# feihuzhang/GANet

Measured on AMD Instinct MI355X. Metric: cost-volumes/sec (SGA+LGA fwd+bwd) at 240x624x192, higher is better.
Workload: dtype f32; 1 GPU; configs[1]: SGA fwd+bwd [1,32,65,80,208] (4x guidance [1,32,5,80,208]) + LGA2 r=2 fwd+bwd [1,193,240,624] (filters [1,75,240,624]), one sample per GPU; parallelism=independent cost volumes per GPU, no data-path collective, launch=hipGraph replay

## Files before the change

### ganet_amd/_native.py

```python
import ctypes
import os
import threading

_HERE = os.path.dirname(os.path.abspath(__file__))
LIB_NAME = "libganet_hip.so"
ABI_VERSION = 11

_P = ctypes.c_void_p
_I = ctypes.c_int

_PROTOS = {
    "ganet_abi_version": [],
    "ganet_is_simulator": [],
    "ganet_set_option": [ctypes.c_char_p, _I],
    "ganet_get_option": [ctypes.c_char_p],
    "ganet_sga_scan_forward": [_P, _P, _P, _I, _I, _I, _I, _I, _I, _P],
    "ganet_sga_forward": [_P] * 9 + [_I] * 5 + [_P],
    "ganet_sga_forward_infer": [_P] * 9 + [_I] * 5 + [_P],
    "ganet_sga_forward_infer_scratch": [_P] * 6 + [_I] * 5,
    "ganet_sga_backward_scan": [_P] * 5 + [_I] * 6 + [_P],
    "ganet_sga_merge": [_P] * 4 + [_I] * 5 + [_P],
    "ganet_sga_scan_forward_ws": [_P] * 3 + [_I] * 6 + [_P],
    "ganet_sga_backward_scan_ws": [_P] * 5 + [_I] * 6 + [_P],
    "ganet_sga_workspace_layout": [_I] * 5,
    "ganet_sga_backward_point": [_P] * 12 + [_I] * 5 + [_P],
    "ganet_sga_backward_dir": [_P] * 9 + [_I] * 7 + [_P],
    "ganet_sga_backward": [_P] * 15 + [_I] * 5 + [_P],
    "ganet_sga_forward_compat": [_P] * 8 + [_I] * 5 + [_P],
    "ganet_sga_backward_compat": [_P] * 15 + [_I] * 5 + [_P],
    "ganet_lga_forward": [_P] * 3 + [_I] * 5 + [_P],
    "ganet_lga_backward": [_P] * 5 + [_I] * 6 + [_P],
    "ganet_lga_forward_regress": [_P] * 5 + [_I] * 5 + [_P],
    "ganet_lga_apply_paired": [_P] * 3 + [_I] * 8 + [_P],
    "ganet_lga_apply_paired_edges": [_P] * 4 + [_I] * 8 + [_P],
    "ganet_lga_filter_grad_paired": [_P] * 3 + [_I] * 8 + [_P],
    "ganet_cost_volume_forward": [_P] * 3 + [_I] * 5 + [_P],
    "ganet_cost_volume_backward": [_P] * 3 + [_I] * 5 + [_P],
    "ganet_disparity_regression_forward": [_P] * 2 + [_I] * 4 + [_P],
    "ganet_disparity_regression_backward": [_P] * 2 + [_I] * 4 + [_P],
    "ganet_l1_normalize_forward": [_P] * 5 + [_I] * 6 + [_P],
    "ganet_l1_normalize_backward": [_P] * 6 + [_I] * 6 + [_P],
    "ganet_norm_disparity_regression_forward": [_P] * 3 + [_I] * 4 + [_P],
    "ganet_norm_disparity_regression_backward": [_P] * 5 + [_I] * 4 + [_P],
    "ganet_softmin_forward": [_P] * 2 + [_I] * 4 + [_P],
    "ganet_softmin_backward": [_P] * 3 + [_I] * 4 + [_P],
    "ganet_softmin_regression_forward": [_P] * 4 + [_I] * 4 + [_P],
    "ganet_softmin_regression_backward": [_P] * 6 + [_I] * 4 + [_P],
    "ganet_trilinear_upsample_forward": [_P] * 2 + [_I] * 7 + [_P],
    "ganet_trilinear_upsample_backward": [_P] * 2 + [_I] * 7 + [_P],
    "ganet_residual_relu_forward": [_P] * 5 + [_I] * 5 + [_P],
    "ganet_residual_relu_backward": [_P] * 5 + [_I] * 5 + [_P],
    "ganet_selftest_dpp": [_P, _P, _P],
    "ganet_selftest_dpp_wave": [_P, _P, _P],
}
EXPORTS = sorted(list(_PROTOS) + ["ganet_last_error"])


class GanetError(RuntimeError):

    def __init__(self, message, code=None):
        super().__init__(message)
        self.code = code


E_INVALID, E_UNSUPPORTED, E_RUNTIME = -1, -2, -3


class CApi:
# ... 68 lines not shown
```

### ganet_amd/csrc/ganet_capi.hip

```cpp
#include "ga_common.h"
#include "lga_kernels.h"
#include "misc_kernels.h"
#include "sga_kernels.h"
#include "sga_row_kernels.h"
#include "sga_col_kernels.h"

#include <stdarg.h>
#include <stdio.h>
#include <stdlib.h>
#include <string.h>

#include <atomic>
#include <mutex>

#include "../../include/ganet_hip.h"

#include "ga_launch.h"

namespace {

using namespace ga;

thread_local char g_err[512] = "";

int fail(int code, const char *fmt, ...)
{
  va_list ap;
  va_start(ap, fmt);
  vsnprintf(g_err, sizeof(g_err), fmt, ap);
  va_end(ap);
  return code;
}

int check_launch(const char *what)
{
  const hipError_t e = hipGetLastError();
  if (e != hipSuccess) return fail(GANET_E_RUNTIME, "%s: %s", what, hipGetErrorString(e));
  return GANET_OK;
}

#define GA_TRY(expr)                         \
  do {                                       \
    const int rc_ = (expr);                  \
    if (rc_ != GANET_OK) return rc_;         \
  } while (0)

#define GA_HIP(expr)                                                                   \
  do {                                                                                 \
    const hipError_t e_ = (expr);                                                      \
    if (e_ != hipSuccess) return fail(GANET_E_RUNTIME, #expr ": %s", hipGetErrorString(e_)); \
  } while (0)

#ifndef GA_SGA_TILED_DEFAULT
#define GA_SGA_TILED_DEFAULT 1
#endif
struct Options {
  std::atomic<int> sga_tiled{GA_SGA_TILED_DEFAULT};
  std::atomic<int> lga_wave{2};
  std::atomic<int> lga_mix{1};
  std::atomic<int> lga_segs{0};
  std::atomic<int> wide_col{1};
  std::atomic<int> wide_scan{1};
  std::atomic<int> rowwave{1};
  std::atomic<int> colblock{1};
};
Options g_opt;
std::once_flag g_opt_once;

bool store_option(const char *name, int value)
{
  auto tri = [](int v) { return v < 0 ? 0 : (v > 2 ? 2 : v); };
  if (!strcmp(name, "GANET_LGA_WAVE")) g_opt.lga_wave = tri(value);
  else if (!strcmp(name, "GANET_SGA_TILED")) g_opt.sga_tiled = value ? 1 : 0;
  else if (!strcmp(name, "GANET_LGA_MIX")) g_opt.lga_mix = value < 0 ? 0 : value;
  else if (!strcmp(name, "GANET_LGA_SEGS")) g_opt.lga_segs = value > 0 ? value : 0;
  else if (!strcmp(name, "GANET_SGA_WIDE_SCAN")) g_opt.wide_scan = tri(value);
  else if (!strcmp(name, "GANET_SGA_WIDE_COL")) g_opt.wide_col = tri(value);
  else if (!strcmp(name, "GANET_SGA_ROWWAVE")) g_opt.rowwave = value ? 1 : 0;
  else if (!strcmp(name, "GANET_SGA_COLBLOCK")) g_opt.colblock = value ? 1 : 0;
  else return false;
  return true;
}

void load_env_options()
{
  for (const char *name : {"GANET_LGA_WAVE", "GANET_SGA_TILED", "GANET_LGA_SEGS", "GANET_LGA_MIX", "GANET_SGA_WIDE_SCAN",
                           "GANET_SGA_WIDE_COL", "GANET_SGA_ROWWAVE", "GANET_SGA_COLBLOCK"}) {
    const char *v = getenv(name);
    if (v && *v) store_option(name, atoi(v));
  }
}
const Options &opts()
{
  std::call_once(g_opt_once, load_env_options);
  return g_opt;
}

#define GA_SGA_PAIRS(X) \
  X(16, 1) X(16, 2) X(16, 3) X(16, 5) X(16, 9) X(16, 13) X(16, 17) \
  X(64, 3) X(64, 5) X(64, 9) X(64, 17)

constexpr int fwd_sb(int dpl) { return dpl <= 3 ? 8 : dpl <= 5 ? 4 : dpl <= 9 ? 2 : 1; }
constexpr int fwd_nv(int dpl) { return dpl <= 5 ? 2 : 1; }
constexpr int bwd_sb(int dpl) { return dpl <= 3 ? 8 : dpl <= 5 ? 4 : dpl <= 9 ? 2 : 1; }
constexpr int bwd_nv(int dpl) { return dpl <= 5 ? 2 : 1; }

bool pick_pair(int D, int want_gd, int *gd, int *dpl)
{
  int best_gd = 0, best_dpl = 0;
#define X(G, P)                                                                    \
  if ((G) == want_gd && (G) * (P) >= D && (best_gd == 0 || (P) < best_dpl)) {      \
    best_gd = (G);                                                                 \
    best_dpl = (P);                                                                \
  }
  GA_SGA_PAIRS(X)
#undef X
  if (best_gd == 0 && want_gd == 16) return pick_pair(D, 64, gd, dpl);
  if (best_gd == 0) return false;
  *gd = best_gd;
  *dpl = best_dpl;
// ... 378 lines not shown
    nseg = tiles * 2 > slots ? 1 : (int)((slots + tiles - 1) / tiles);
    if (nseg > D / 16) nseg = D / 16 > 1 ? D / 16 : 1;
  }
  if (nseg > D) nseg = D;
  if (nseg > 1) {
    mx.n_whole = 0;
    mx.sub_len = ((D + nseg - 1) / nseg + 1) & ~1;
    mx.nsub = (D + mx.sub_len - 1) / mx.sub_len;
    *items = tiles * mx.nsub;
    return mx;
  }
  const int mixo = opts().lga_mix;
  const i64 S = mixo > 1 ? (i64)mixo : (i64)units;
  if (mixo && opts().lga_segs <= 0 && tiles / S < LGA_WAVES_PER_SIMD && tiles % S != 0) {
    const i64 r = tiles % S;
    int nsub = (int)(S / r);
    if (nsub > D / 16) nsub = D / 16;
    if (nsub >= 2) {
      mx.n_whole = (int)(tiles - r);
      mx.sub_len = ((D + nsub - 1) / nsub + 1) & ~1;
      mx.nsub = (D + mx.sub_len - 1) / mx.sub_len;
      *items = mx.n_whole + r * mx.nsub;
    }
  }
  return mx;
}

#ifndef GA_LGA_PLANAR
#ifndef GA_FGP_DEFAULT
#define GA_FGP_DEFAULT 1
#endif
#ifndef GA_FGP_WPS
#define GA_FGP_WPS 5
#endif
#define GA_LGA_PLANAR 1
#endif
template <int R>
int launch_lga_fwd(const float *x, const float *f, float *y, int B, int D, int H, int W,
                   bool transposed, hipStream_t st)
{
  LgaGeom geo;
  geo.D = D; geo.H = H; geo.W = W; geo.HW = (i64)H * W;
  if constexpr (R <= 2) {
    const int family = opts().lga_wave;
    if (family && (i64)H * W < (1ll << 28)) {
      i64 items;
      bool planar = false;
      if constexpr (R == 2) planar = GA_LGA_PLANAR && W % 4 == 0 && aligned16(x);
      if constexpr (R == 2) {
        if (planar && family == 2) {
          const LgaSegMix wx = lga_items(W, H, B, D, false, &items, true);
          if (items < (1ll << 31)) {
            if (transposed) GA_LAUNCH((lga_apply_pp_wx<2, true>), dim3((unsigned)items), dim3(256), st, x, f, y, geo, wx);
            else GA_LAUNCH((lga_apply_pp_wx<2, false>), dim3((unsigned)items), dim3(256), st, x, f, y, geo, wx);
            return check_launch("lga apply (plane pairs, workgroup ring)");
          }
        }
      }
      const LgaSegMix mx = lga_items(W, H, B, D, false, &items);
      if (items < (1ll << 31)) {
        if constexpr (R == 2) {
          if (planar && transposed) GA_LAUNCH((lga_apply_pp_x<2, true>), dim3((unsigned)items), dim3(64), st, x, f, y, geo, mx);
          else if (planar) GA_LAUNCH((lga_apply_pp_x<2, false>), dim3((unsigned)items), dim3(64), st, x, f, y, geo, mx);
        }
        if (planar) {}
        else if (transposed) GA_LAUNCH((lga_apply_pp<R, true>), dim3((unsigned)items), dim3(64), st, x, f, y, geo, mx);
// ... 41 lines not shown
#define L(K, T) GA_LAUNCH((K<2, T>), dim3((unsigned)items), dim3(64), st, x, f, y, geo, sg, none, none, edge)
  if (x_paired) {
    if (transposed) L(lga_apply_pp_pi, true); else L(lga_apply_pp_pi, false);
  } else if (GA_LGA_PLANAR && W % 4 == 0) {
    if (transposed) L(lga_apply_pp_xo, true); else L(lga_apply_pp_xo, false);
  } else {
    if (transposed) L(lga_apply_pp_po, true); else L(lga_apply_pp_po, false);
  }
#undef L
  return check_launch("lga apply (plane pairs, interleaved volume)");
}

int launch_lga_gf_paired(const float *x, const float *gy, float *gf, int B, int D, int H, int W, int acc, bool x_paired,
                         hipStream_t st)
{
  if ((i64)H * W >= (1ll << 28) || W % 2 != 0 || !aligned16(x) || !aligned16(gy))
    return fail(GANET_E_UNSUPPORTED, "ganet_lga_filter_grad_paired: needs W even, planes below 2^28 pixels and 16-byte aligned volumes");
  LgaGeom geo;
  geo.D = D; geo.H = H; geo.W = W; geo.HW = (i64)H * W;
  LgaSeg sg;
  sg.tiles_x = (W + LGA_TW - 1) / LGA_TW;
  sg.tiles_y = (H + LGAW_TH - 1) / LGAW_TH;
  sg.nseg = 1; sg.seg_len = D;
  const i64 items = (i64)sg.tiles_x * sg.tiles_y * B;
  if (items >= (1ll << 31)) return fail(GANET_E_UNSUPPORTED, "ganet_lga_filter_grad_paired: too many tiles");
  const bool fg_pair = GA_FGP_DEFAULT && opts().lga_wave >= 2;
  if (x_paired && fg_pair) GA_LAUNCH((lga_filter_grad_pair_xp<GA_FGP_WPS>), dim3((unsigned)items), dim3(128), st, x, gy, gf, geo, sg, acc);
  else if (x_paired) GA_LAUNCH((lga_filter_grad_pp_xp<2, 3, 0>), dim3((unsigned)items), dim3(64), st, x, gy, gf, geo, sg, acc);
  else if (GA_LGA_PLANAR && W % 4 == 0) GA_LAUNCH((lga_filter_grad_pp_gypx<2, 3, 0>), dim3((unsigned)items), dim3(64), st, x, gy, gf, geo, sg, acc);
  else GA_LAUNCH((lga_filter_grad_pp_gyp<2, 3, 0>), dim3((unsigned)items), dim3(64), st, x, gy, gf, geo, sg, acc);
  return check_launch("lga filter grad (plane pairs, interleaved volume)");
}

template <int R>
int launch_lga_fwd_regress(const float *x, const float *f, float *y, float *snorm, float *sdy, int B, int D, int H, int W,
                           hipStream_t st)
{
  if constexpr (R <= 2) {
    if ((i64)H * W < (1ll << 28)) {
      LgaGeom geo;
      geo.D = D; geo.H = H; geo.W = W; geo.HW = (i64)H * W;
      i64 items;
      const LgaSegMix sg = lga_items(W, H, B, D, true, &items);
      if (items < (1ll << 31)) {
        bool planar = false;
        if constexpr (R == 2) {
          planar = GA_LGA_PLANAR && W % 4 == 0 && aligned16(x);
          if (planar) GA_LAUNCH((lga_apply_pp_x<2, false, true>), dim3((unsigned)items), dim3(64), st, x, f, y, geo, sg, snorm, sdy);
        }
        if (!planar) GA_LAUNCH((lga_apply_pp<R, false, true>), dim3((unsigned)items), dim3(64), st, x, f, y, geo, sg, snorm, sdy);
        return check_launch("lga apply + regression epilogue (plane pairs)");
      }
    }
  }
  return fail(GANET_E_UNSUPPORTED, "ganet_lga_forward_regress: no fused kernel for this shape / radius: run ganet_lga_forward "
                                   "and ganet_norm_disparity_regression_forward instead");
}

template <int R>
int launch_lga_gf(const float *x, const float *gy, float *gf, int B, int D, int H, int W, int acc,
                  hipStream_t st)
{
  LgaGeom geo;
  geo.D = D; geo.H = H; geo.W = W; geo.HW = (i64)H * W;
  if constexpr (R <= 2) {
    if (opts().lga_wave && (i64)H * W < (1ll << 28)) {
// ... 48 lines not shown
{
  const int lane = threadIdx.x;
  out[0 * 64 + lane] = dpp_i<DPP_WAVE_SHL1>(-1, lane);
  out[1 * 64 + lane] = dpp_i<DPP_WAVE_SHR1>(-1, lane);
  out[2 * 64 + lane] = (int)seg_allmax<64>((float)((lane * 37) % 64));
  out[3 * 64 + lane] = (int)seg_allsum<64>((float)lane);
}

}

GA_EXPORT int ganet_abi_version(void) { return GANET_ABI_VERSION; }
GA_EXPORT const char *ganet_last_error(void) { return g_err; }
GA_EXPORT int ganet_is_simulator(void)
{
#if defined(GA_HIPSIM)
  return 1;
#else
  return 0;
#endif
}

GA_EXPORT int ganet_get_option(const char *name)
{
  opts();
  if (!name) return fail(GANET_E_INVALID, "ganet_get_option: null name");
  if (!strcmp(name, "GANET_LGA_WAVE")) return g_opt.lga_wave;
  if (!strcmp(name, "GANET_SGA_TILED")) return g_opt.sga_tiled;
  if (!strcmp(name, "GANET_LGA_MIX")) return g_opt.lga_mix;
  if (!strcmp(name, "GANET_LGA_SEGS")) return g_opt.lga_segs;
  if (!strcmp(name, "GANET_SGA_WIDE_SCAN")) return g_opt.wide_scan;
  if (!strcmp(name, "GANET_SGA_WIDE_COL")) return g_opt.wide_col;
  if (!strcmp(name, "GANET_SGA_ROWWAVE")) return g_opt.rowwave;
  if (!strcmp(name, "GANET_SGA_COLBLOCK")) return g_opt.colblock;
  return fail(GANET_E_INVALID, "ganet_get_option: unknown option %s", name);
}

GA_EXPORT int ganet_set_option(const char *name, int value)
{
  opts();
  if (!name) return fail(GANET_E_INVALID, "ganet_set_option: null name");
  if (store_option(name, value)) {}
#if defined(GA_HIPSIM)
  else if (!strcmp(name, "HIPSIM_LATE_DMA")) hipsim::S().late_dma = value != 0;
  else if (!strcmp(name, "HIPSIM_LANE_ORDER")) hipsim::S().lane_order = value ? 1 : 0;
  else if (!strcmp(name, "HIPSIM_WAVE_GREEDY")) hipsim::S().wave_greedy = value ? 1 : 0;
  else if (!strcmp(name, "HIPSIM_LATE_LDS")) hipsim::S().late_lds = value != 0;
  else if (!strcmp(name, "HIPSIM_LGKM_SLACK")) hipsim::S().lgkm_slack = value;
  else if (!strcmp(name, "HIPSIM_VMCNT_SLACK")) hipsim::S().vm_slack = value;
#endif
  else {
    static const char *const retired[] = {"GANET_LGA_BWD_STREAMS", "GANET_LGA_FG_WPS", "GANET_LGA_SPLIT", "GANET_LGA_VMCNT_SAFE",
                                          "GANET_SGA_BLOCK_H", "GANET_SGA_BLOCK_V", "GANET_SGA_GD", "GANET_SGA_GD_H", "GANET_SGA_GD_V",
                                          "GANET_SGA_INFER_FUSED", "GANET_SGA_MERGE4", "GANET_SGA_POINT_BLOCK", "GANET_SGA_STREAMS",
                                          "GANET_LGA_WG", "GANET_SGA_POINT_Q4"};
    for (const char *r : retired)
      if (!strcmp(name, r)) {
        static std::atomic<int> noted{0};
        if (!noted.exchange(1)) fprintf(stderr, "[ganet] ganet_set_option: %s is retired (no effect); see INTEGRATION.md\n", name);
        return GANET_OK;
      }
    return fail(GANET_E_INVALID, "ganet_set_option: unknown option %s", name);
  }
  return GANET_OK;
}

GA_EXPORT int ganet_sga_scan_forward(const float *x, const float *g, float *A, int N, int C, int D,
// ... 267 lines not shown
  GA_TRY(check_lga(who, B, D, H, W, radius));
  if (x_paired && y_paired) return fail(GANET_E_INVALID, "%s: at most one of x_paired / y_paired", who);
  if (radius != 2) return fail(GANET_E_UNSUPPORTED, "%s: radius 2 only", who);
  if (!x_paired && !y_paired) {
    if (edge) return fail(GANET_E_UNSUPPORTED, "%s: the edge-sum side channel belongs to the pair-interleaved forms", who);
    return launch_lga_fwd<2>(x, f, y, B, D, H, W, transposed != 0, (hipStream_t)stream);
  }
  return launch_lga_paired(x, f, y, B, D, H, W, transposed != 0, x_paired != 0, (hipStream_t)stream, edge);
}
}

GA_EXPORT int ganet_lga_apply_paired(const float *x, const float *f, float *y, int B, int D, int H, int W, int radius,
                                     int transposed, int x_paired, int y_paired, void *stream)
{
  return lga_apply_paired_impl("ganet_lga_apply_paired", x, f, y, nullptr, B, D, H, W, radius, transposed, x_paired, y_paired, stream);
}

GA_EXPORT int ganet_lga_apply_paired_edges(const float *x, const float *f, float *y, float *edge, int B, int D, int H, int W, int radius,
                                           int transposed, int x_paired, int y_paired, void *stream)
{
  if (!edge) return fail(GANET_E_INVALID, "ganet_lga_apply_paired_edges: null edge buffer");
  return lga_apply_paired_impl("ganet_lga_apply_paired_edges", x, f, y, edge, B, D, H, W, radius, transposed, x_paired, y_paired, stream);
}

GA_EXPORT int ganet_lga_filter_grad_paired(const float *x, const float *gy, float *gf, int B, int D, int H, int W, int radius,
                                           int accumulate_gf, int x_paired, int gy_paired, void *stream)
{
  if (!x || !gy || !gf) return fail(GANET_E_INVALID, "ganet_lga_filter_grad_paired: null pointer");
  GA_TRY(check_lga("ganet_lga_filter_grad_paired", B, D, H, W, radius));
  if (x_paired && gy_paired) return fail(GANET_E_INVALID, "ganet_lga_filter_grad_paired: at most one of x_paired / gy_paired");
  if (radius != 2) return fail(GANET_E_UNSUPPORTED, "ganet_lga_filter_grad_paired: radius 2 only");
  if (!x_paired && !gy_paired) return launch_lga_gf<2>(x, gy, gf, B, D, H, W, accumulate_gf != 0, (hipStream_t)stream);
  return launch_lga_gf_paired(x, gy, gf, B, D, H, W, accumulate_gf != 0, x_paired != 0, (hipStream_t)stream);
}

GA_EXPORT int ganet_lga_forward_regress(const float *x, const float *f, float *y, float *snorm, float *sdy, int B, int D,
                                        int H, int W, int radius, void *stream)
{
  if (!x || !f || !snorm || !sdy) return fail(GANET_E_INVALID, "ganet_lga_forward_regress: null pointer");
  if (x == y) return fail(GANET_E_INVALID, "ganet_lga_forward_regress: y must not alias x");
  GA_TRY(check_lga("ganet_lga_forward_regress", B, D, H, W, radius));
  hipStream_t st = (hipStream_t)stream;
  if (radius == 1) return launch_lga_fwd_regress<1>(x, f, y, snorm, sdy, B, D, H, W, st);
  if (radius == 2) return launch_lga_fwd_regress<2>(x, f, y, snorm, sdy, B, D, H, W, st);
  return launch_lga_fwd_regress<3>(x, f, y, snorm, sdy, B, D, H, W, st);
}

GA_EXPORT int ganet_lga_backward(const float *x, const float *f, const float *gy, float *gx,
                                 float *gf, int B, int D, int H, int W, int radius,
                                 int accumulate_gf, void *stream)
{
  if (!x || !f || !gy || !gx || !gf) return fail(GANET_E_INVALID, "ganet_lga_backward: null pointer");
  if (gx == gy) return fail(GANET_E_INVALID, "ganet_lga_backward: gx must not alias gy");
  GA_TRY(check_lga("ganet_lga_backward", B, D, H, W, radius));
  hipStream_t st = (hipStream_t)stream;
  const int acc = accumulate_gf ? 1 : 0;
  int rc;
  if (radius == 1) { rc = launch_lga_gf<1>(x, gy, gf, B, D, H, W, acc, st); if (rc == GANET_OK) rc = launch_lga_fwd<1>(gy, f, gx, B, D, H, W, true, st); }
  else if (radius == 2) { rc = launch_lga_gf<2>(x, gy, gf, B, D, H, W, acc, st); if (rc == GANET_OK) rc = launch_lga_fwd<2>(gy, f, gx, B, D, H, W, true, st); }
  else { rc = launch_lga_gf<3>(x, gy, gf, B, D, H, W, acc, st); if (rc == GANET_OK) rc = launch_lga_fwd<3>(gy, f, gx, B, D, H, W, true, st); }
  return rc;
}

GA_EXPORT int ganet_cost_volume_forward(const float *x, const float *y, float *cost, int N, int C,
                                        int Dn, int H, int W, void *stream)
{
// ... 333 lines not shown
```

### ganet_amd/csrc/lga_kernels.h

```cpp
#pragma once
#include "ga_common.h"
#include <type_traits>

namespace ga {

constexpr int LGA_TW = 32;
constexpr int LGA_TH = 8;
constexpr int LGA_NT = LGA_TW * LGA_TH;
constexpr int LGA_PB = 4;
#ifndef LGA_WAVES_PER_SIMD
#define LGA_WAVES_PER_SIMD 3
#endif

template <int R> struct LgaCfg {
  static constexpr int WS = 2 * R + 1;
  static constexpr int K = WS * WS;
  static constexpr int RE = (R + 1) & ~1;
  static constexpr int NP = R + 1;
  static constexpr int NK = 2 * NP;
  static constexpr int TW2 = LGA_TW + 2 * RE;
  static constexpr int TH2 = LGA_TH + 2 * R;
  static constexpr int PLANE = TW2 * TH2;
  static constexpr int STAGE = PLANE * LGA_PB;
  static constexpr int NLD = (STAGE + LGA_NT - 1) / LGA_NT;
// ... 720 lines not shown
#define GA_FG_NDC ND
#include "lga_filter_grad_pp.inc"
#define GA_FG_NAME lga_filter_grad_pp_x
#define GA_FG_XP 2
#define GA_FG_GYP 0
#define GA_FG_SLOT 512
#define GA_FG_NDC 2
#include "lga_filter_grad_pp.inc"
#define GA_FG_NAME lga_filter_grad_pp_xp
#define GA_FG_XP 1
#define GA_FG_GYP 0
#define GA_FG_SLOT 512
#define GA_FG_NDC 2
#include "lga_filter_grad_pp.inc"

#define GA_FG_NAME lga_filter_grad_pp_gyp
#define GA_FG_XP 0
#define GA_FG_GYP 1
#define GA_FG_SLOT PC::SLOT
#define GA_FG_NDC ND
#include "lga_filter_grad_pp.inc"
#define GA_FG_NAME lga_filter_grad_pp_gypx
#define GA_FG_XP 2
#define GA_FG_GYP 1
#define GA_FG_SLOT 512
#define GA_FG_NDC 2
#include "lga_filter_grad_pp.inc"

#define GA_FGP_NAME lga_filter_grad_pair_xp
#define GA_FGP_XP 1
#define GA_FGP_GYP 0
#include "lga_filter_grad_pair.inc"

template <int R>
__global__ void __launch_bounds__(LGA_NT, (R <= 2 ? LGA_WAVES_PER_SIMD : 1))
lga_filter_grad(const float *__restrict__ x, const float *__restrict__ gy, float *__restrict__ gf,
                LgaGeom geo, int accumulate)
{
  typedef LgaCfg<R> C;
  __shared__ __attribute__((aligned(16))) float tile[2][C::STAGE];
  const int tx = threadIdx.x % LGA_TW, ty = threadIdx.x / LGA_TW;
  int bx, by, b;
  {
    const int nb = gridDim.x * gridDim.y * gridDim.z;
    const int lid = xcd_remap(blockIdx.x + gridDim.x * (blockIdx.y + gridDim.y * blockIdx.z), nb);
    bx = lid % gridDim.x;
    by = (lid / gridDim.x) % gridDim.y;
    b = lid / (gridDim.x * gridDim.y);
  }
  const int tx0 = bx * LGA_TW, ty0 = by * LGA_TH;
  const int i = ty0 + ty, j = tx0 + tx;
  const bool inb = i < geo.H && j < geo.W;
  const int ic = i < geo.H ? i : geo.H - 1, jc = j < geo.W ? j : geo.W - 1;
  const float *xb = x + (i64)b * geo.D * geo.HW;
  const float *gyb = gy + (i64)b * geo.D * geo.HW;
  float *gfb = gf + (i64)b * 3 * C::K * geo.HW;
  const i64 pix = (i64)ic * geo.W + jc;
  const int wcol = tx + C::RE - R;
  const int par = wcol & 1;
  const int rcol = wcol - par;

  f2 sab[C::WS][C::NK], sc[C::WS][C::NP];
#pragma unroll
  for (int a = 0; a < C::WS; a++) {
#pragma unroll
    for (int k = 0; k < C::NK; k++) sab[a][k] = mk2(0.f, 0.f);
// ... 108 lines not shown
```

### ganet_amd/functions/GANet.py

```python
import os

import torch
from torch.autograd import Function

from .. import _native

__all__ = ["SgaFunction", "LgaFunction", "Lga2Function", "Lga3Function", "Lga3dFunction",
           "Lga3d2Function", "Lga3d3Function", "Lgf2Function", "MyLossFunction", "MyLoss2Function",
           "GetCostVolumeFunction", "DisparityRegressionFunction"]


def _lib():
    return _native.lib()


def _check(*tensors):
    dev = tensors[0].device
    for t in tensors:
        if not t.is_cuda:
            raise RuntimeError("ganet_amd ops need HIP (cuda) tensors: there is no CPU path")
        if t.dtype != torch.float32:
            raise TypeError(f"ganet_amd ops are fp32 only, got {t.dtype}")
        if t.device != dev:
            raise RuntimeError("all tensors of a ganet_amd op must live on one device")
# ... 123 lines not shown
                        _lib().call("ganet_lga_apply_paired", _p(input), _p(filters), _p(t1p), B, D, H, W, radius, 0, 0, 1, _stream())
                    _lib().call("ganet_lga_apply_paired", _p(t1p), _p(filters), _p(y), B, D, H, W, radius, 0, 1, 0, _stream())
                    ctx.paired = True
                except _native.GanetError as e:
                    if e.code != _native.E_UNSUPPORTED:
                        raise
            if ctx.paired:
                ctx.edge = edge
                ctx.save_for_backward(filters, input, t1p)
                return y
        ins = [input]
        with torch.cuda.device_of(input):
            for _ in range(cls.passes):
                y = torch.empty_like(input)
                _lib().call("ganet_lga_forward", _p(ins[-1]), _p(filters), _p(y), B, D, H, W, radius, _stream())
                ins.append(y)
        ctx.save_for_backward(filters, *ins[:-1])
        return ins[-1]

    @staticmethod
    def _bwd(ctx, gradOutput):
        filters, *ins = ctx.saved_tensors
        g = gradOutput.contiguous()
        if getattr(ctx, "paired", False) and g.data_ptr() % 16 != 0:
            g = g.clone(memory_format=torch.contiguous_format)
        _check(g)
        B, D, H, W = _lga_dims(ins[0], filters, ctx.radius)
        if getattr(ctx, "paired", False):
            x, t1p = ins
            with torch.cuda.device_of(g):
                gradFilters = torch.empty_like(filters)
                gt1p, gx = torch.empty_like(t1p), torch.empty_like(x)
                lib, st, r = _lib(), _stream(), ctx.radius
                lib.call("ganet_lga_filter_grad_paired", _p(t1p), _p(g), _p(gradFilters), B, D, H, W, r, 0, 1, 0, st)
                edge = getattr(ctx, "edge", None)
                if edge is not None:
                    lib.call("ganet_lga_apply_paired_edges", _p(g), _p(filters), _p(gt1p), _p(edge), B, D, H, W, r, 1, 0, 1, st)
                else:
                    lib.call("ganet_lga_apply_paired", _p(g), _p(filters), _p(gt1p), B, D, H, W, r, 1, 0, 1, st)
                lib.call("ganet_lga_filter_grad_paired", _p(x), _p(gt1p), _p(gradFilters), B, D, H, W, r, 1, 0, 1, st)
                if edge is not None:
                    lib.call("ganet_lga_apply_paired_edges", _p(gt1p), _p(filters), _p(gx), _p(edge), B, D, H, W, r, 1, 1, 0, st)
                else:
                    lib.call("ganet_lga_apply_paired", _p(gt1p), _p(filters), _p(gx), B, D, H, W, r, 1, 1, 0, st)
            return gx, gradFilters, None
        with torch.cuda.device_of(g):
            gradFilters = torch.empty_like(filters)
            for k, xin in enumerate(reversed(ins)):
                gx = torch.empty_like(xin)
                _lib().call("ganet_lga_backward", _p(xin), _p(filters), _p(g), _p(gx), _p(gradFilters),
                            B, D, H, W, ctx.radius, 1 if k > 0 else 0, _stream())
                g = gx
        return g, gradFilters, None


def _make_lga(name, passes, doc):
    def forward(ctx, input, filters, radius=1):
        return cls._fwd(ctx, input, filters, radius)

    def backward(ctx, gradOutput):
        return _LgaChain._bwd(ctx, gradOutput)

    cls = type(name, (_LgaChain,), {"passes": passes, "__doc__": doc,
                                    "forward": staticmethod(forward), "backward": staticmethod(backward)})
    return cls


LgaFunction = _make_lga("LgaFunction", 1, "one LGA pass on [N,D,H,W] (functions/GANet.py:239-263)")
Lga2Function = _make_lga("Lga2Function", 2, "two chained passes (functions/GANet.py:174-203); what the models use")
Lga3Function = _make_lga("Lga3Function", 3, "three chained passes (functions/GANet.py:141-173)")
Lga3dFunction = _make_lga("Lga3dFunction", 1, "one pass per (n,c) on [N,C,D,H,W] (functions/GANet.py:115-139)")
Lga3d2Function = _make_lga("Lga3d2Function", 2, "two passes, 5-D (functions/GANet.py:84-113)")
Lga3d3Function = _make_lga("Lga3d3Function", 3, "three passes, 5-D (functions/GANet.py:51-83)")
Lgf2Function = Lga2Function


class GetCostVolumeFunction(Function):
# ... 101 lines not shown
```

### include/ganet_hip.h

```cpp
#ifndef GANET_HIP_H
#define GANET_HIP_H

#include <stdint.h>

#ifdef __cplusplus
extern "C" {
#endif

#define GANET_OK 0
#define GANET_E_INVALID (-1)
#define GANET_E_UNSUPPORTED (-2)
#define GANET_E_RUNTIME (-3)

#define GANET_ABI_VERSION 11
int ganet_abi_version(void);
const char *ganet_last_error(void);
int ganet_is_simulator(void);


int ganet_sga_scan_forward(const float *x, const float *g, float *A,
                           int N, int C, int D, int H, int W, int dir, void *stream);

int ganet_sga_forward(const float *x, const float *g0, const float *g1, const float *g2,
                      const float *g3, float *A_ws, float *out, uint8_t *mask, uint16_t *kp,
                      int N, int C, int D, int H, int W, void *stream);

int ganet_sga_scan_forward_ws(const float *x, const float *g, float *A_ws,
                              int N, int C, int D, int H, int W, int dir, void *stream);
int ganet_sga_backward_scan_ws(const float *g, const uint8_t *mask, const uint16_t *kp, const float *grad_out, float *G_ws,
                               int N, int C, int D, int H, int W, int dir, void *stream);
int ganet_sga_workspace_layout(int N, int C, int D, int H, int W);

int ganet_sga_merge(const float *A_ws, float *out, uint8_t *mask, uint16_t *kp,
                    int N, int C, int D, int H, int W, void *stream);

int ganet_sga_forward_infer(const float *x, const float *g0, const float *g1, const float *g2,
                            const float *g3, float *A_ws, float *out, const float *bn_scale,
                            const float *bn_shift, int N, int C, int D, int H, int W, void *stream);
int ganet_sga_forward_infer_scratch(const float *x, const float *g0, const float *g1, const float *g2,
                                    const float *g3, const float *out, int N, int C, int D, int H, int W);

int ganet_sga_backward_scan(const float *g, const uint8_t *mask, const uint16_t *kp_dir,
                            const float *grad_out, float *G,
                            int N, int C, int D, int H, int W, int dir, void *stream);

int ganet_sga_backward_dir(const float *x, const float *g, const float *A, const uint8_t *mask,
                           const uint16_t *kp_dir, const float *grad_out, float *G_ws,
// ... 4 lines not shown
int ganet_sga_backward(const float *x, const float *g0, const float *g1, const float *g2,
                       const float *g3, const float *A_ws, const uint8_t *mask, const uint16_t *kp,
                       const float *grad_out, float *G_ws, float *grad_x, float *gw0, float *gw1,
                       float *gw2, float *gw3, int N, int C, int D, int H, int W, void *stream);

int ganet_sga_backward_point(const float *x, const float *g0, const float *g1, const float *g2, const float *g3,
                             const float *A_ws, const float *G_ws, float *grad_x, float *gw0, float *gw1,
                             float *gw2, float *gw3, int N, int C, int D, int H, int W, void *stream);

int ganet_sga_forward_compat(const float *x, const float *g0, const float *g1, const float *g2,
                             const float *g3, float *temp_out, float *out, float *mask_f32,
                             int N, int C, int D, int H, int W, void *stream);
int ganet_sga_backward_compat(const float *x, const float *g0, const float *g1, const float *g2,
                              const float *g3, float *temp_out, const float *mask_f32,
                              float *max_idx, const float *grad_out, float *temp_grad,
                              float *grad_x, float *gw0, float *gw1, float *gw2, float *gw3,
                              int N, int C, int D, int H, int W, void *stream);


int ganet_lga_forward(const float *x, const float *f, float *y,
                      int B, int D, int H, int W, int radius, void *stream);

int ganet_lga_forward_regress(const float *x, const float *f, float *y, float *snorm, float *sdy,
                              int B, int D, int H, int W, int radius, void *stream);

int ganet_lga_apply_paired(const float *x, const float *f, float *y, int B, int D, int H, int W, int radius,
                           int transposed, int x_paired, int y_paired, void *stream);
int ganet_lga_apply_paired_edges(const float *x, const float *f, float *y, float *edge, int B, int D, int H, int W, int radius,
                                 int transposed, int x_paired, int y_paired, void *stream);

int ganet_lga_filter_grad_paired(const float *x, const float *gy, float *gf, int B, int D, int H, int W, int radius,
                                 int accumulate_gf, int x_paired, int gy_paired, void *stream);

int ganet_lga_backward(const float *x, const float *f, const float *gy, float *gx, float *gf,
                       int B, int D, int H, int W, int radius, int accumulate_gf, void *stream);


int ganet_cost_volume_forward(const float *x, const float *y, float *cost,
                              int N, int C, int Dn, int H, int W, void *stream);
int ganet_cost_volume_backward(const float *grad_cost, float *grad_x, float *grad_y,
                               int N, int C, int Dn, int H, int W, void *stream);

int ganet_disparity_regression_forward(const float *x, float *out,
                                       int N, int Dn, int H, int W, void *stream);
int ganet_disparity_regression_backward(const float *grad_out, float *grad_x,
                                        int N, int Dn, int H, int W, void *stream);


int ganet_l1_normalize_forward(const float *x, float *y0, float *y1, float *y2, float *y3,
                               int N, int G, int C, int K, int H, int W, void *stream);
int ganet_l1_normalize_backward(const float *x, const float *gy0, const float *gy1,
                                const float *gy2, const float *gy3, float *grad_x,
                                int N, int G, int C, int K, int H, int W, void *stream);

int ganet_norm_disparity_regression_forward(const float *x, float *out, float *snorm,
                                            int N, int Dn, int H, int W, void *stream);
int ganet_norm_disparity_regression_backward(const float *x, const float *out, const float *snorm,
                                             const float *grad_out, float *grad_x,
                                             int N, int Dn, int H, int W, void *stream);

int ganet_softmin_forward(const float *x, float *y, int N, int Dn, int H, int W, void *stream);
int ganet_softmin_backward(const float *y, const float *grad_y, float *grad_x,
                           int N, int Dn, int H, int W, void *stream);

int ganet_softmin_regression_forward(const float *x, float *out, float *mx, float *ssum,
                                     int N, int Dn, int H, int W, void *stream);
// ... 26 lines not shown
```

Measured before the change: 658.7 cost-volumes/sec.

## Fuse LGA backward data-gradient and filter-gradient into one two-wave kernel

Adds a fused LGA backward kernel in which one wave of each block computes the data gradient (applying filters to the paired gy) while the other wave accumulates the filter gradient from x and the same gy tile in shared memory. The second of the two LGA2 backward stages (gy paired, gx unpaired) now goes through this kernel, so gy is loaded once for both outputs and one launch is saved. The fused path is taken only when there are enough tiles to fill the device several times over. Otherwise it falls back to the separate filter-grad and apply calls. The first stage always uses the fallback. Giving each half of the work its own wave may cost occupancy and leave waves idle if the two halves are not balanced.

After: 658.0 cost-volumes/sec (median of 3 runs). No clear change (-0.1%).

```diff
diff --git a/ganet_amd/_native.py b/ganet_amd/_native.py
--- a/ganet_amd/_native.py
+++ b/ganet_amd/_native.py
@@ -4,7 +4,7 @@
 
 _HERE = os.path.dirname(os.path.abspath(__file__))
 LIB_NAME = "libganet_hip.so"
-ABI_VERSION = 11
+ABI_VERSION = 12
 
 _P = ctypes.c_void_p
 _I = ctypes.c_int
@@ -34,6 +34,7 @@
     "ganet_lga_apply_paired": [_P] * 3 + [_I] * 8 + [_P],
     "ganet_lga_apply_paired_edges": [_P] * 4 + [_I] * 8 + [_P],
     "ganet_lga_filter_grad_paired": [_P] * 3 + [_I] * 8 + [_P],
+    "ganet_lga_backward_paired": [_P] * 6 + [_I] * 9 + [_P],
     "ganet_cost_volume_forward": [_P] * 3 + [_I] * 5 + [_P],
     "ganet_cost_volume_backward": [_P] * 3 + [_I] * 5 + [_P],
     "ganet_disparity_regression_forward": [_P] * 2 + [_I] * 4 + [_P],
diff --git a/ganet_amd/csrc/ganet_capi.hip b/ganet_amd/csrc/ganet_capi.hip
--- a/ganet_amd/csrc/ganet_capi.hip
+++ b/ganet_amd/csrc/ganet_capi.hip
@@ -53,6 +53,9 @@
 
 #ifndef GA_SGA_TILED_DEFAULT
 #define GA_SGA_TILED_DEFAULT 1
+#endif
+#ifndef GA_LGA_BWD_PASS_DEFAULT
+#define GA_LGA_BWD_PASS_DEFAULT 1
 #endif
 struct Options {
   std::atomic<int> sga_tiled{GA_SGA_TILED_DEFAULT};
@@ -63,6 +66,7 @@
   std::atomic<int> wide_scan{1};
   std::atomic<int> rowwave{1};
   std::atomic<int> colblock{1};
+  std::atomic<int> lga_bwd_pass{GA_LGA_BWD_PASS_DEFAULT};
 };
 Options g_opt;
 std::once_flag g_opt_once;
@@ -78,6 +82,7 @@
   else if (!strcmp(name, "GANET_SGA_WIDE_COL")) g_opt.wide_col = tri(value);
   else if (!strcmp(name, "GANET_SGA_ROWWAVE")) g_opt.rowwave = value ? 1 : 0;
   else if (!strcmp(name, "GANET_SGA_COLBLOCK")) g_opt.colblock = value ? 1 : 0;
+  else if (!strcmp(name, "GANET_LGA_BWD_PASS")) g_opt.lga_bwd_pass = tri(value);
   else return false;
   return true;
 }
@@ -85,7 +90,7 @@
 void load_env_options()
 {
   for (const char *name : {"GANET_LGA_WAVE", "GANET_SGA_TILED", "GANET_LGA_SEGS", "GANET_LGA_MIX", "GANET_SGA_WIDE_SCAN",
-                           "GANET_SGA_WIDE_COL", "GANET_SGA_ROWWAVE", "GANET_SGA_COLBLOCK"}) {
+                           "GANET_SGA_WIDE_COL", "GANET_SGA_ROWWAVE", "GANET_SGA_COLBLOCK", "GANET_LGA_BWD_PASS"}) {
     const char *v = getenv(name);
     if (v && *v) store_option(name, atoi(v));
   }
@@ -530,6 +535,9 @@
 #endif
 #ifndef GA_FGP_WPS
 #define GA_FGP_WPS 5
+#endif
+#ifndef GA_BWD_PASS_WPS
+#define GA_BWD_PASS_WPS 3
 #endif
 #define GA_LGA_PLANAR 1
 #endif
@@ -637,6 +645,34 @@
   return check_launch("lga filter grad (plane pairs, interleaved volume)");
 }
 
+bool lga_bwd_pass_fused(const float *x, const float *gy, const float *gx, const float *edge, int B, int H, int W, int radius,
+                        int x_paired, int gy_paired, int gx_paired)
+{
+  const int mode = opts().lga_bwd_pass;
+  if (mode == 0 || !(radius == 2 && opts().lga_wave == 2 && !x_paired && gy_paired && !gx_paired && edge != nullptr && W % 4 == 0 &&
+                     (i64)H * W < (1ll << 28) && aligned16(x) && aligned16(gy) && aligned16(gx)))
+    return false;
+  const i64 tiles = (i64)((W + LGA_TW - 1) / LGA_TW) * ((H + LGAW_TH - 1) / LGAW_TH) * B;
+  const i64 resident = (i64)device_cus() * 4 * GA_BWD_PASS_WPS / 2;
+  return mode == 2 || tiles >= 3 * resident;
+}
+
+int launch_lga_bwd_pass(const float *x, const float *gy, const float *f, const float *edge, float *gx, float *gf, int B, int D, int H,
+                        int W, int acc, hipStream_t st)
+{
+  LgaGeom geo;
+  geo.D = D; geo.H = H; geo.W = W; geo.HW = (i64)H * W;
+  LgaSeg sg;
+  sg.tiles_x = (W + LGA_TW - 1) / LGA_TW;
+  sg.tiles_y = (H + LGAW_TH - 1) / LGAW_TH;
+  sg.nseg = 1; sg.seg_len = D;
+  const i64 items = (i64)sg.tiles_x * sg.tiles_y * B;
+  if (items >= (1ll << 31)) return fail(GANET_E_UNSUPPORTED, "ganet_lga_backward_paired: too many tiles");
+  GA_LAUNCH((lga_bwd_pass_gyp<GA_BWD_PASS_WPS>), dim3((unsigned)items), dim3(128), st, x, gy, f, edge, gx, gf, geo, sg, acc);
+  if (getenv("GANET_TRACE_DISPATCH")) fprintf(stderr, "[ganet] lga_bwd_pass_gyp items=%lld\n", (long long)items);
+  return check_launch("lga backward pass (data-backward + filter gradient, one launch)");
+}
+
 template <int R>
 int launch_lga_fwd_regress(const float *x, const float *f, float *y, float *snorm, float *sdy, int B, int D, int H, int W,
                            hipStream_t st)
@@ -751,6 +787,7 @@
   if (!strcmp(name, "GANET_SGA_WIDE_COL")) return g_opt.wide_col;
   if (!strcmp(name, "GANET_SGA_ROWWAVE")) return g_opt.rowwave;
   if (!strcmp(name, "GANET_SGA_COLBLOCK")) return g_opt.colblock;
+  if (!strcmp(name, "GANET_LGA_BWD_PASS")) return g_opt.lga_bwd_pass;
   return fail(GANET_E_INVALID, "ganet_get_option: unknown option %s", name);
 }
 
@@ -1084,6 +1121,22 @@
   if (radius != 2) return fail(GANET_E_UNSUPPORTED, "ganet_lga_filter_grad_paired: radius 2 only");
   if (!x_paired && !gy_paired) return launch_lga_gf<2>(x, gy, gf, B, D, H, W, accumulate_gf != 0, (hipStream_t)stream);
   return launch_lga_gf_paired(x, gy, gf, B, D, H, W, accumulate_gf != 0, x_paired != 0, (hipStream_t)stream);
+}
+
+GA_EXPORT int ganet_lga_backward_paired(const float *x, const float *gy, const float *f, float *edge, float *gx, float *gf, int B, int D,
+                                        int H, int W, int radius, int accumulate_gf, int x_paired, int gy_paired, int gx_paired,
+                                        void *stream)
+{
+  if (!x || !gy || !f || !gx || !gf) return fail(GANET_E_INVALID, "ganet_lga_backward_paired: null pointer");
+  if (gx == gy) return fail(GANET_E_INVALID, "ganet_lga_backward_paired: gx must not alias gy");
+  GA_TRY(check_lga("ganet_lga_backward_paired", B, D, H, W, radius));
+  if (x_paired && gy_paired) return fail(GANET_E_INVALID, "ganet_lga_backward_paired: at most one of x_paired / gy_paired");
+  if (gy_paired && gx_paired) return fail(GANET_E_INVALID, "ganet_lga_backward_paired: at most one of gy_paired / gx_paired");
+  if (lga_bwd_pass_fused(x, gy, gx, edge, B, H, W, radius, x_paired, gy_paired, gx_paired))
+    return launch_lga_bwd_pass(x, gy, f, edge, gx, gf, B, D, H, W, accumulate_gf != 0, (hipStream_t)stream);
+  GA_TRY(ganet_lga_filter_grad_paired(x, gy, gf, B, D, H, W, radius, accumulate_gf, x_paired, gy_paired, stream));
+  if (edge) return ganet_lga_apply_paired_edges(gy, f, gx, edge, B, D, H, W, radius, 1, gy_paired, gx_paired, stream);
+  return ganet_lga_apply_paired(gy, f, gx, B, D, H, W, radius, 1, gy_paired, gx_paired, stream);
 }
 
 GA_EXPORT int ganet_lga_forward_regress(const float *x, const float *f, float *y, float *snorm, float *sdy, int B, int D,
diff --git a/ganet_amd/csrc/lga_bwd_pass.inc b/ganet_amd/csrc/lga_bwd_pass.inc
--- /dev/null
+++ b/ganet_amd/csrc/lga_bwd_pass.inc
@@ -0,0 +1,371 @@
+template <int WPS>
+__global__ void __launch_bounds__(128, WPS)
+lga_bwd_pass_gyp(const float *__restrict__ x, const float *__restrict__ gy, const float *__restrict__ f, const float *__restrict__ edge,
+                 float *__restrict__ gx, float *__restrict__ gf, LgaGeom geo, LgaSeg sg, int accumulate)
+{
+  constexpr int R = 2;
+  typedef LgaPCfg<R> PC;
+  constexpr int WS = PC::WS, K = WS * WS, NR = LGAP_NR, P = NR - 1, SLOT = 512, NDC = 2;
+  constexpr int LA = LGAW_LA;
+  constexpr int U = (WS % (LA + 1) == 0) ? 1 : (LA + 1);
+  static_assert(P >= 2 && NDC * P < 64, "vmcnt immediate");
+  static_assert(PC::TH2 * PC::TW2 * 2 <= SLOT && PC::TW2 % 2 == 0 && PC::TH2 * (PC::TW2 / 2) <= 128, "two 16-byte copies per gy pair");
+  __shared__ __attribute__((aligned(16))) float gring[NR * SLOT];
+  __shared__ __attribute__((aligned(16))) float xring[NR * SLOT];
+  __shared__ float edge_sums[2 * 64];
+  const int lane = threadIdx.x & 63;
+  const int part = GA_UNIFORM_I((int)(threadIdx.x >> 6));
+  const int tx = lane % LGA_TW, ty = lane / LGA_TW;
+  int item = xcd_remap(blockIdx.x, gridDim.x);
+  const int bx = item % sg.tiles_x; item /= sg.tiles_x;
+  const int by = item % sg.tiles_y;
+  const int b = item / sg.tiles_y;
+  const int tx0 = bx * LGA_TW, ty0 = by * LGAW_TH;
+  const int i = ty0 + ty, j = tx0 + tx;
+  const int ic = i < geo.H ? i : geo.H - 1, jc = j < geo.W ? j : geo.W - 1;
+  const int D = geo.D;
+  const int npair = (D + 1) >> 1;
+  const int nsteps = U * ((npair + U - 1) / U);
+  auto next_slot = [](int off) { return off + SLOT == NR * SLOT ? 0 : off + SLOT; };
+
+  if (part == 0) {
+    const bool inb = i < geo.H && j < geo.W;
+    const float *xb = gy + (i64)b * npair * 2 * geo.HW;
+    const float *fb = f + (i64)b * 3 * K * geo.HW;
+    float *yb = gx + (i64)b * geo.D * geo.HW;
+    const int pix = ic * geo.W + jc;
+    unsigned goff[2];
+#pragma unroll
+    for (int k = 0; k < 2; k++) {
+      constexpr int NPIECE = PC::TH2 * (PC::TW2 / 2);
+      int piece = k * 64 + lane;
+      piece = piece < NPIECE ? piece : NPIECE - 1;
+      const int r = piece / (PC::TW2 / 2), c = 2 * (piece - r * (PC::TW2 / 2));
+      int i2 = ty0 + r - R, j2 = tx0 + c - R;
+      i2 = i2 < 0 ? 0 : (i2 < geo.H ? i2 : geo.H - 1);
+      j2 = j2 < 0 ? 0 : (j2 < geo.W - 1 ? j2 : geo.W - 2);
+      goff[k] = 8u * (unsigned)(i2 * geo.W + j2) + LGAP_BIAS - 1024u * (unsigned)k;
+    }
+    const float *gbase = reinterpret_cast<const float *>(reinterpret_cast<const char *>(xb) - LGAP_BIAS);
+    int soff_d = 0;
+    auto dma = [&](int q) {
+      lga_dma16p_pair(gbase, goff, gring + soff_d, lane);
+      if (q + 1 < npair) gbase += 2 * geo.HW;
+    };
+    for (int q = 0; q < P; q++) { dma(q); soff_d = next_slot(soff_d); }
+
+    constexpr int NT = 3 * K, NWP = (NT + 1) / 2;
+    f2 wq[NWP];
+    float cmid = 0.f;
+    {
+      float sin_m0 = 0.f, sin_p0 = 0.f;
+      const bool interior = ty0 >= R && ty0 + LGAW_TH + R <= geo.H && tx0 >= R && tx0 + LGA_TW + R <= geo.W;
+      const float *ep = edge + (i64)b * 3 * geo.HW + pix;
+      cmid = ep[0]; sin_m0 = ep[geo.HW]; sin_p0 = ep[2 * geo.HW];
+      if (interior)
+        lga_gather_pairs<R, true, false, false>(fb, geo, ic, jc, wq, cmid, sin_m0, sin_p0);
+      else
+        lga_gather_pairs<R, true, true, false>(fb, geo, ic, jc, wq, cmid, sin_m0, sin_p0);
+      edge_sums[lane] = sin_m0;
+      edge_sums[64 + lane] = sin_p0;
+    }
+
+    constexpr int ROWF = 2 * PC::TW2;
+    const lds_cptr lbase = GA_LDS_CPTR(&gring[0]) + 2 * (ty * PC::TW2 + tx);
+    auto read_row = [&](f2 (&row)[WS], int t, lds_cptr cur, lds_cptr nxt) {
+      const lds_cptr src = t < WS ? cur + t * ROWF : nxt + (t - WS) * ROWF;
+#pragma unroll
+      for (int bb = 0; bb < WS; bb++) row[bb] = lds_read_b64(src + 2 * bb);
+    };
+    f2 vrow[LA + 1][WS];
+    GA_VMCNT(0);
+    GA_LDS_BARRIER();
+#pragma unroll
+    for (int s0 = 0; s0 < LA; s0++) read_row(vrow[s0], s0, lbase, lbase);
+
+    f2 o_prev = mk2(0.f, 0.f);
+    float e_hi_prev = 0.f;
+    float xc_prev = 0.f;
+    int soff_c = 0;
+    constexpr int NSTEP = U * WS;
+    static_assert(NSTEP % (LA + 1) == 0, "row ring must close");
+    float *yp = yb;
+    const unsigned ypix = 4u * (unsigned)pix;
+#define GA_BP_YP(T) reinterpret_cast<T *>(reinterpret_cast<char *>(yp) + ypix)
+    auto group = [&](auto steady_tag, int q0) {
+      constexpr bool STEADY = decltype(steady_tag)::value;
+      f2 eA, eB, pA, pB, cA, cB;
+      float sin_m = 0.f, sin_p = 0.f;
+      if (!STEADY) { sin_m = edge_sums[lane]; sin_p = edge_sums[64 + lane]; }
+      f2 xc2 = mk2(0.f, 0.f);
+#pragma unroll
+      for (int st = 0; st < NSTEP; st++) {
+        const int u = st / WS, a = st % WS;
+        const int q = q0 + u;
+        const int m = q;
+        if (a == 0) {
+          GA_VMCNT(NDC * (P - 2));
+          GA_LDS_BARRIER();
+          if (STEADY) {
+            lga_dma16p_pair(gbase, goff, gring + soff_d, lane);
+            gbase += 2 * geo.HW;
+          } else {
+            dma(q + P);
+          }
+          soff_d = next_slot(soff_d);
+        }
+        const int soff_n = soff_c + SLOT == NR * SLOT ? 0 : soff_c + SLOT;
+        const lds_cptr cur = lbase + soff_c, nxt = lbase + soff_n;
+        read_row(vrow[(st + LA) % (LA + 1)], a + LA, cur, nxt);
+        GA_SCHED_FENCE();
+        {
+          const f2 (&Xr)[WS] = vrow[st % (LA + 1)];
+          const f2 *We = &wq[(K + a * WS) >> 1], *Wp = &wq[(2 * K + a * WS) >> 1], *Wc = &wq[(a * WS) >> 1];
+          if (a == 0) lga_row_fma<false, true, -1>(eA, pA, cA, eB, pB, cB, Xr, We, Wp, Wc);
+          else if (a & 1) lga_row_fma<true, false, -1>(eB, pB, cB, eA, pA, cA, Xr, We, Wp, Wc);
+          else lga_row_fma<false, false, -1>(eA, pA, cA, eB, pB, cB, Xr, We, Wp, Wc);
+          if (a == R) xc2 = Xr[R];
+        }
+        if (a == WS - 1) {
+          GA_KEEP_F2(eA); GA_KEEP_F2(eB); GA_KEEP_F2(pA); GA_KEEP_F2(pB); GA_KEEP_F2(cA); GA_KEEP_F2(cB);
+          const f2 e = add2(eA, eB);
+          const f2 o = add2(o_prev, add2(pA, pB));
+          if (STEADY) {
+            const float r1 = fmaf(xc_prev, cmid, e_hi_prev + o.x);
+            const float r2 = fmaf(xc2.x, cmid, e.x + o.y);
+            if (inb) stream_store<(GA_NT_STORES & 16) != 0 || (GA_NT_STORES & 64) != 0>(GA_BP_YP(float), r1);
+            yp += geo.HW;
+            if (inb) stream_store<(GA_NT_STORES & 16) != 0 || (GA_NT_STORES & 64) != 0>(GA_BP_YP(float), r2);
+            yp += geo.HW;
+            o_prev = add2(cA, cB);
+            e_hi_prev = e.y;
+            xc_prev = xc2.y;
+          } else {
+            const bool live = q < npair;
+            const int d1 = 2 * m - 1, d2 = 2 * m;
+            if (live && d1 >= 0 && d1 < D) {
+              float cc = cmid;
+              if (d1 == D - 1) cc += sin_p;
+              const float r = fmaf(xc_prev, cc, e_hi_prev + o.x);
+              if (inb) yb[(i64)d1 * geo.HW + pix] = r;
+            }
+            if (live && d2 >= 0 && d2 < D) {
+              float cc = cmid;
+              if (d2 == 0) cc += sin_m;
+              if (d2 == D - 1) cc += sin_p;
+              const float r = fmaf(xc2.x, cc, e.x + o.y);
+              if (inb) yb[(i64)d2 * geo.HW + pix] = r;
+            }
+            if (live) {
+              o_prev = add2(cA, cB);
+              e_hi_prev = e.y;
+              xc_prev = xc2.y;
+            }
+          }
+          soff_c = soff_n;
+        }
+      }
+    };
+    const int ql = 1;
+    int qh = npair - P - 1;
+    if ((D >> 1) - P < qh) qh = (D >> 1) - P;
+    {
+      const int L = D - 1;
+      if (((L + 1) >> 1) < qh) qh = (L + 1) >> 1;
+    }
+    int q0 = 0;
+    for (; q0 < npair && q0 < ql; q0 += U) group(std::false_type{}, q0);
+    if (q0 + U <= qh) yp = yb + (i64)(2 * q0 - 1) * geo.HW;
+    for (; q0 + U <= qh; q0 += U) group(std::true_type{}, q0);
+    for (; q0 < npair; q0 += U) group(std::false_type{}, q0);
+    {
+      const int d1 = 2 * ((D - 1) >> 1) + 1;
+      const float sin_p = edge_sums[64 + lane];
+      if (d1 < D) {
+        float cc = cmid;
+        if (d1 == D - 1) cc += sin_p;
+        const float r = fmaf(xc_prev, cc, e_hi_prev + o_prev.x);
+        if (inb) yb[(i64)d1 * geo.HW + pix] = r;
+      }
+    }
+    GA_VMCNT(0);
+#undef GA_BP_YP
+  } else {
+    const float *xb = x + (i64)b * geo.D * geo.HW;
+    constexpr int TWL = LGA_TW + 8, NCH = TWL / 4, NPIECE = PC::TH2 * 2 * NCH;
+    static_assert(NPIECE <= 128 && PC::TH2 * 2 * TWL <= SLOT, "two 16-byte copies per pair");
+    auto piece_odd = [&](int k) { int piece = k * 64 + lane; piece = piece < NPIECE ? piece : NPIECE - 1; return ((piece / NCH) & 1) != 0; };
+    unsigned goff[2];
+#pragma unroll
+    for (int k = 0; k < 2; k++) {
+      int piece = k * 64 + lane;
+      piece = piece < NPIECE ? piece : NPIECE - 1;
+      const int r = piece / (2 * NCH), pl = (piece / NCH) & 1, c = 4 * (piece % NCH);
+      int i2 = ty0 + r - R, j2 = tx0 + c - 4;
+      i2 = i2 < 0 ? 0 : (i2 < geo.H ? i2 : geo.H - 1);
+      j2 = j2 < 0 ? 0 : (j2 < geo.W - 3 ? j2 : geo.W - 4);
+      goff[k] = 4u * ((unsigned)pl * (unsigned)geo.HW + (unsigned)(i2 * geo.W + j2)) + LGAP_BIAS - 1024u * (unsigned)k;
+    }
+    const float *xsrc = reinterpret_cast<const float *>(reinterpret_cast<const char *>(xb) - LGAP_BIAS);
+    auto dma_x = [&](int q, int soff_d) {
+      const int qq = q < npair ? q : npair - 1;
+      const bool half = 2 * qq + 1 >= D;
+      float *slot = xring + soff_d;
+      if (half) {
+        unsigned ge[2];
+#pragma unroll
+        for (int k = 0; k < 2; k++) ge[k] = piece_odd(k) ? goff[k] - 4u * (unsigned)geo.HW : goff[k];
+        lga_dma16p_pair(xsrc, ge, slot, lane);
+        if (q < npair) {
+          GA_VMCNT(0);
+          GA_WAVE_SYNC();
+#pragma unroll
+          for (int k = 0; k < 2; k++)
+            if (piece_odd(k)) *reinterpret_cast<f4 *>(slot + k * 256 + 4 * lane) = f4{0.f, 0.f, 0.f, 0.f};
+          GA_LGKMCNT0();
+          GA_WAVE_SYNC();
+        }
+      } else {
+        lga_dma16p_pair(xsrc, goff, slot, lane);
+      }
+      if (q + 1 < npair) xsrc += 2 * geo.HW;
+    };
+    for (int q = 0; q < P; q++) dma_x(q, q * SLOT);
+
+    f2 Pq[WS][WS], Qq[WS][WS];
+#pragma unroll
+    for (int a = 0; a < WS; a++) {
+#pragma unroll
+      for (int bb = 0; bb < WS; bb++) Pq[a][bb] = Qq[a][bb] = mk2(0.f, 0.f);
+    }
+    float gc = 0.f;
+    float e_lo = 0.f, e_hi = 0.f;
+    float g_odd = 0.f;
+    constexpr int ROWF = 2 * TWL;
+    const lds_cptr lbase = GA_LDS_CPTR(&xring[0]) + ty * ROWF + tx + (4 - R);
+    const lds_cptr gcell = GA_LDS_CPTR(&gring[0]) + 2 * ((ty + R) * PC::TW2 + tx + R);
+    auto read_row = [&](f2 (&row)[WS], int t, lds_cptr cur) {
+      const lds_cptr cur3 = cur + 3 * ROWF;
+      switch (t) {
+        case 0: lds_read2_row5<0, ROWF, TWL>(row, cur); break;
+        case 1: lds_read2_row5<1, ROWF, TWL>(row, cur); break;
+        case 2: lds_read2_row5<2, ROWF, TWL>(row, cur); break;
+        case 3: lds_read2_row5<0, ROWF, TWL>(row, cur3); break;
+        default: lds_read2_row5<1, ROWF, TWL>(row, cur3); break;
+      }
+    };
+    GA_VMCNT(0);
+    GA_LDS_BARRIER();
+    int soff_c = 0;
+    int soff_d = (P % NR) * SLOT;
+    auto step = [&](auto steady_tag, auto phase_tag, int q) {
+      constexpr bool STEADY = decltype(steady_tag)::value;
+      constexpr int PH = decltype(phase_tag)::value;
+      const int xs_c = PH >= 0 ? ((1 + PH) % NR) * SLOT : soff_c;
+      const int xs_n = PH >= 0 ? ((2 + PH) % NR) * SLOT : next_slot(soff_c);
+      const int xs_d = PH >= 0 ? ((1 + PH + P) % NR) * SLOT : soff_d;
+      GA_WAVE_SYNC();
+      if (STEADY) {
+        lga_dma16p_pair(xsrc, goff, xring + xs_d, lane);
+        xsrc += 2 * geo.HW;
+        GA_OPAQUE_S(xsrc);
+      } else {
+        dma_x(q + P, xs_d);
+      }
+      GA_VMCNT(NDC * P);
+      GA_LDS_BARRIER();
+      const f2 A = lds_read_b64(gcell + xs_c);
+      const f2 Bn = lds_read_b64(gcell + xs_n);
+      const f2 Ov = mk2(g_odd, A.x);
+      const f2 Nv = mk2(A.y, Bn.x);
+      g_odd = A.y;
+      f2 Gc, Gn;
+      if (STEADY) {
+        Gc = Ov;
+        Gn = Nv;
+      } else {
+        Gc = mk2(q > 0 ? Ov.x : 0.f, Ov.y);
+        Gn = mk2(2 * q + 1 < D ? Nv.x : 0.f, 2 * q + 2 < D ? Nv.y : 0.f);
+      }
+      const f2 Ga = mk2(Gn.x, Gc.y);
+      f2 xc2 = mk2(0.f, 0.f);
+      const lds_cptr cur = lbase + xs_c;
+#pragma unroll
+      for (int a = 0; a < WS; a++) {
+        f2 row[WS];
+        read_row(row, a, cur);
+        GA_SCHED_FENCE();
+        lga_row_fg<0>(Pq[a], Qq[a], row, Ga, Gn, Gc);
+        if (a == R) xc2 = row[R];
+        GA_SCHED_FENCE();
+      }
+      {
+        const float e0 = Ga.y * xc2.x, e1 = Ga.x * xc2.y;
+        gc += e0 + e1;
+        if (!STEADY) {
+          if (q == 0) e_lo = e0;
+          if (2 * q == D - 1) e_hi = e0;
+          if (2 * q + 1 == D - 1) e_hi = e1;
+        }
+      }
+      if (PH < 0) {
+        soff_c = next_slot(soff_c);
+        soff_d = next_slot(soff_d);
+      }
+    };
+    auto steady_group = [&](int q0) {
+      step(std::true_type{}, std::integral_constant<int, 0>{}, q0);
+      if constexpr (NR > 1) step(std::true_type{}, std::integral_constant<int, 1>{}, q0 + 1);
+      if constexpr (NR > 2) step(std::true_type{}, std::integral_constant<int, 2>{}, q0 + 2);
+      if constexpr (NR > 3) step(std::true_type{}, std::integral_constant<int, 3>{}, q0 + 3);
+      if constexpr (NR > 4) step(std::true_type{}, std::integral_constant<int, 4>{}, q0 + 4);
+      if constexpr (NR > 5) step(std::true_type{}, std::integral_constant<int, 5>{}, q0 + 5);
+      static_assert(NR <= 6, "steady_group is written out for up to six ring slots");
+    };
+    int qh = (D - 2 - 2 * P) >> 1;
+    if (npair - P - 1 < qh) qh = npair - P - 1;
+    int q0 = 0;
+    const auto rt = std::integral_constant<int, -1>{};
+    for (; q0 < npair && q0 < 1; q0++) step(std::false_type{}, rt, q0);
+    for (; q0 + NR <= qh; q0 += NR) steady_group(q0);
+    for (; q0 < npair; q0++) step(std::false_type{}, rt, q0);
+    for (int s = npair; s < nsteps; s++) GA_LDS_BARRIER();
+    GA_VMCNT(0);
+
+    {
+      int lane2 = lane;
+#if !defined(GA_HIPSIM)
+      asm volatile("" : "+v"(lane2));
+#endif
+      const int i_ = ty0 + lane2 / LGA_TW, j_ = tx0 + lane2 % LGA_TW;
+      if (i_ < geo.H && j_ < geo.W) {
+        float *gfp = gf + (i64)b * 3 * K * geo.HW + (i64)i_ * geo.W + j_;
+#pragma unroll
+        for (int dd = 0; dd < 3; dd++) {
+          float old[K];
+#pragma unroll
+          for (int k = 0; k < K; k++) old[k] = 0.f;
+          if (accumulate) {
+#pragma unroll
+            for (int k = 0; k < K; k++) old[k] = gfp[(i64)(dd * K + k) * geo.HW];
+          }
+#pragma unroll
+          for (int a = -R; a <= R; a++) {
+#pragma unroll
+            for (int bb = -R; bb <= R; bb++) {
+              const int t = dd * K + (a + R) * WS + (bb + R);
+              const int i2 = i_ + a, j2 = j_ + bb;
+              const bool ok = i2 >= 0 && i2 < geo.H && j2 >= 0 && j2 < geo.W;
+              float r;
+              if (dd == 0) r = Pq[a + R][bb + R].x + e_lo;
+              else if (dd == 1) r = Pq[a + R][bb + R].y;
+              else r = Qq[a + R][bb + R].x + Qq[a + R][bb + R].y + e_hi;
+              if (!ok) r = gc;
+              stream_store<(GA_NT_STORES & 32) != 0>(gfp + (i64)t * geo.HW, old[(a + R) * WS + (bb + R)] + r);
+            }
+          }
+        }
+      }
+    }
+  }
+}
diff --git a/ganet_amd/csrc/lga_kernels.h b/ganet_amd/csrc/lga_kernels.h
--- a/ganet_amd/csrc/lga_kernels.h
+++ b/ganet_amd/csrc/lga_kernels.h
@@ -776,6 +776,8 @@
 #define GA_FGP_GYP 0
 #include "lga_filter_grad_pair.inc"
 
+#include "lga_bwd_pass.inc"
+
 template <int R>
 __global__ void __launch_bounds__(LGA_NT, (R <= 2 ? LGA_WAVES_PER_SIMD : 1))
 lga_filter_grad(const float *__restrict__ x, const float *__restrict__ gy, float *__restrict__ gf,
diff --git a/ganet_amd/functions/GANet.py b/ganet_amd/functions/GANet.py
--- a/ganet_amd/functions/GANet.py
+++ b/ganet_amd/functions/GANet.py
@@ -179,17 +179,12 @@
                 gradFilters = torch.empty_like(filters)
                 gt1p, gx = torch.empty_like(t1p), torch.empty_like(x)
                 lib, st, r = _lib(), _stream(), ctx.radius
-                lib.call("ganet_lga_filter_grad_paired", _p(t1p), _p(g), _p(gradFilters), B, D, H, W, r, 0, 1, 0, st)
                 edge = getattr(ctx, "edge", None)
-                if edge is not None:
-                    lib.call("ganet_lga_apply_paired_edges", _p(g), _p(filters), _p(gt1p), _p(edge), B, D, H, W, r, 1, 0, 1, st)
-                else:
-                    lib.call("ganet_lga_apply_paired", _p(g), _p(filters), _p(gt1p), B, D, H, W, r, 1, 0, 1, st)
-                lib.call("ganet_lga_filter_grad_paired", _p(x), _p(gt1p), _p(gradFilters), B, D, H, W, r, 1, 0, 1, st)
-                if edge is not None:
-                    lib.call("ganet_lga_apply_paired_edges", _p(gt1p), _p(filters), _p(gx), _p(edge), B, D, H, W, r, 1, 1, 0, st)
-                else:
-                    lib.call("ganet_lga_apply_paired", _p(gt1p), _p(filters), _p(gx), B, D, H, W, r, 1, 1, 0, st)
+                ep = _p(edge) if edge is not None else None
+                lib.call("ganet_lga_backward_paired", _p(t1p), _p(g), _p(filters), ep, _p(gt1p), _p(gradFilters),
+                         B, D, H, W, r, 0, 1, 0, 1, st)
+                lib.call("ganet_lga_backward_paired", _p(x), _p(gt1p), _p(filters), ep, _p(gx), _p(gradFilters),
+                         B, D, H, W, r, 1, 0, 1, 0, st)
             return gx, gradFilters, None
         with torch.cuda.device_of(g):
             gradFilters = torch.empty_like(filters)
diff --git a/include/ganet_hip.h b/include/ganet_hip.h
--- a/include/ganet_hip.h
+++ b/include/ganet_hip.h
@@ -12,7 +12,7 @@
 #define GANET_E_UNSUPPORTED (-2)
 #define GANET_E_RUNTIME (-3)
 
-#define GANET_ABI_VERSION 11
+#define GANET_ABI_VERSION 12
 int ganet_abi_version(void);
 const char *ganet_last_error(void);
 int ganet_is_simulator(void);
@@ -83,6 +83,9 @@
 int ganet_lga_filter_grad_paired(const float *x, const float *gy, float *gf, int B, int D, int H, int W, int radius,
                                  int accumulate_gf, int x_paired, int gy_paired, void *stream);
 
+int ganet_lga_backward_paired(const float *x, const float *gy, const float *f, float *edge, float *gx, float *gf, int B, int D,
+                              int H, int W, int radius, int accumulate_gf, int x_paired, int gy_paired, int gx_paired, void *stream);
+
 int ganet_lga_backward(const float *x, const float *f, const float *gy, float *gx, float *gf,
                        int B, int D, int H, int W, int radius, int accumulate_gf, void *stream);
 
```
